# nico-franco-gomez/dsptoolbox

Hardware: AMD Instinct MI355X
Metric: Msamples/s + GB/s vs HBM roofline, 64ch Welch H1 nfft=4096 @1/2/4/8 GPU (higher is better)
Workload: dtype f32

## Files before the change

### dsptoolbox_amd/csrc/kernels_welch4096w.hpp

```cpp
#pragma once
#include <utility>

#include "kernels_welch4096.hpp"

namespace welch4096 {

constexpr int L3S = 17;
constexpr int LDS3_BYTES = 16 * L1S * 8 + 256 * 8 + N * 4;

struct Tw6 {
    float2 a[3];
    float2 b[3];
};

__device__ __forceinline__ void load_tw6(Tw6& tw, const float2* __restrict__ twt, int tid) {
#pragma unroll
    for (int j = 0; j < 3; ++j) {
        tw.a[j] = twt[j * 256 + tid];
        tw.b[j] = twt[(4 * (j + 1) - 1) * 256 + tid];
    }
}

__device__ __forceinline__ void apply_tw6(float2 (&v)[16], const Tw6& tw) {
#pragma unroll
    for (int k1 = 1; k1 < 16; ++k1) {
        const int lo = k1 & 3, hi = k1 >> 2;
        float2 z = v[pos16(k1)];
        if (lo) z = cmul(z, tw.a[lo - 1]);
        if (hi) z = cmul(z, tw.b[hi - 1]);
        v[pos16(k1)] = z;
    }
}

__device__ __forceinline__ __amdgpu_buffer_rsrc_t channel_rsrc(const float* ch, int64_t n_samples) {
    return __builtin_amdgcn_make_buffer_rsrc(const_cast<float*>(ch), 0, (int)(uint32_t)(n_samples * 4), 0x00020000);
}
__device__ __forceinline__ float ld_sample(__amdgpu_buffer_rsrc_t r, int byte_off) {
    return __builtin_bit_cast(float, __builtin_amdgcn_raw_buffer_load_b32(r, byte_off, 0, 0));
}

typedef float v2f_t __attribute__((ext_vector_type(2)));
__device__ __forceinline__ uint32_t lds_addr(const void* p) { return (uint32_t)(uintptr_t)p; }
template <int BYTE_OFF>
__device__ __forceinline__ void lds_rd64(float2& d, uint32_t addr) {
    static_assert(BYTE_OFF >= 0 && BYTE_OFF < 65536 && BYTE_OFF % 8 == 0, "ds_read_b64 offset");
    v2f_t r;
    asm volatile("ds_read_b64 %0, %1 offset:%2" : "=v"(r) : "v"(addr), "n"(BYTE_OFF) : "memory");
    d = make_float2(r.x, r.y);
}
template <int N>
__device__ __forceinline__ void lgkm_wait() {
    static_assert(N >= 0 && N <= 15, "lgkmcnt is a 4-bit counter");
    asm volatile("s_waitcnt lgkmcnt(%0)" ::"n"(N) : "memory");
    __builtin_amdgcn_sched_barrier(0);
}
template <typename F, int... I>
__device__ __forceinline__ void static_for_impl(F&& f, std::integer_sequence<int, I...>) {
    (f(std::integral_constant<int, I>{}), ...);
}
template <int N, typename F>
__device__ __forceinline__ void static_for(F&& f) {
    static_for_impl(static_cast<F&&>(f), std::make_integer_sequence<int, N>{});
}

__device__ __forceinline__ int bin_thread(int tid) { return ((tid & 15) << 4) | (tid >> 4); }

template <typename Hook = NoHook, typename Hook2 = NoHook>
__device__ __forceinline__ void fft4096_w(float2 (&v)[16], const Tw6& tw, float2* __restrict__ buf,
                                          const float2* __restrict__ tw2, int tid,
                                          Hook behind_ex1 = Hook(), Hook2 behind_ex2 = Hook2()) {
    dft16(v);
    apply_tw6(v, tw);
    const int k1u = tid >> 4, n3 = tid & 15;
    __syncthreads();
#pragma unroll
    for (int k1 = 0; k1 < 16; ++k1) buf[k1 * L1S + tid] = v[pos16(k1)];
    float2 w2[15];
#pragma unroll
    for (int k2 = 1; k2 < 16; ++k2) w2[k2 - 1] = tw2[k2 * 16 + n3];
    behind_ex1();
    __syncthreads();
    float2* __restrict__ row = buf + k1u * L1S;
#pragma unroll
    for (int n2 = 0; n2 < 16; ++n2) v[n2] = row[16 * n2 + n3];
    dft16(v);
#pragma unroll
    for (int k2 = 1; k2 < 16; ++k2) v[pos16(k2)] = cmul(v[pos16(k2)], w2[k2 - 1]);
#pragma unroll
    for (int k2 = 0; k2 < 16; ++k2) row[n3 * L3S + k2] = v[pos16(k2)];
    behind_ex2();
    wave_sync();
#pragma unroll
    for (int j = 0; j < 16; ++j) v[j] = row[j * L3S + n3];
    dft16(v);
}

__device__ __forceinline__ void set_prio(int level16, int dither) {
    const int pr = min(3, (level16 + dither) >> 2);
    if (pr == 0)
        __builtin_amdgcn_s_setprio(0);
    else if (pr == 1)
        __builtin_amdgcn_s_setprio(1);
    else if (pr == 2)
        __builtin_amdgcn_s_setprio(2);
    else
        __builtin_amdgcn_s_setprio(3);
}

template <typename LA, typename LB, typename MID = NoHook>
__device__ __forceinline__ void fft4096_wi(float2 (&v)[16], const Tw6& tw, float2* __restrict__ buf,
                                           const float2* __restrict__ tw2, int tid, LA ld_a, LB ld_b,
                                           MID mid = MID()) {
    const int k1u = tid >> 4, n3 = tid & 15;
    float2* __restrict__ col = buf + tid;
    dft16_h(
        v, NoHookI(),
        [&](int g) {
            W4_PIN();
            ld_a(g);
            W4_PIN();
        },
        [&](int g) {
#pragma unroll
        for (int j = 0; j < 4; ++j) {
            float2 z = v[4 * g + j];
            if (g) z = cmul(z, tw.a[g - 1]);
            if (j) z = cmul(z, tw.b[j - 1]);
            W4_PIN();
            col[(g + 4 * j) * L1S] = z;
            W4_PIN();
        }
    });
    __syncthreads();
    mid();
    float2* __restrict__ row = buf + k1u * L1S;
    const uint32_t a_row = lds_addr(row + n3), a_tw2 = lds_addr(tw2 + n3);
    W4_PIN();
    static_for<16>([&](auto ic) {
        constexpr int i = decltype(ic)::value, n2 = 4 * (i & 3) + (i >> 2);
        lds_rd64<16 * n2 * 8>(v[n2], a_row);
    });
    float2 w2[16];
    dft16_h(
        v,
        [&](auto gc) {
            constexpr int g = decltype(gc)::value;
            lgkm_wait<(g == 0 ? 12 : 11)>();
        },
        [&](int g) {
            W4_PIN();
            static_for<4>([&](auto jc) {
                constexpr int j = decltype(jc)::value;
                if (g == 0 && j > 0) lds_rd64<(0 + j) * 16 * 8>(w2[0 + j], a_tw2);
                if (g == 1) lds_rd64<(4 + j) * 16 * 8>(w2[4 + j], a_tw2);
                if (g == 2) lds_rd64<(8 + j) * 16 * 8>(w2[8 + j], a_tw2);
                if (g == 3) lds_rd64<(12 + j) * 16 * 8>(w2[12 + j], a_tw2);
            });
            if (g == 3) lgkm_wait<0>();
            W4_PIN();
        },
        [&](int g) {
#pragma unroll
            for (int j = 0; j < 4; ++j) {
                const int k2 = g + 4 * j;
                float2 z = v[4 * g + j];
                if (k2) z = cmul(z, w2[k2]);
                W4_PIN();
                row[n3 * L3S + k2] = z;
                W4_PIN();
            }
            W4_PIN();
            ld_b(g);
            W4_PIN();
        });
    wave_sync();
    W4_PIN();
    static_for<16>([&](auto ic) {
        constexpr int i = decltype(ic)::value, j = 4 * (i & 3) + (i >> 2);
        lds_rd64<j * L3S * 8>(v[j], a_row);
    });
    dft16_h(
        v,
        [&](auto gc) {
            constexpr int g = decltype(gc)::value;
            lgkm_wait<12 - 4 * g>();
            if (g == 3) __syncthreads();
        },
        NoHookI(), NoHookI());
}

struct Tw6R {
    float2 a[3];
    float2 b[3];
    float2 c;
};
constexpr int TW2R = TWT_R + 4 * 256;

__device__ __forceinline__ void load_tw6r(Tw6R& tw, const float2* __restrict__ twt, int tid) {
#pragma unroll
    for (int j = 0; j < 3; ++j) {
        tw.a[j] = twt[TWT_R + j * 256 + tid];
        tw.b[j] = twt[(4 * (j + 1) - 1) * 256 + tid];
    }
    tw.c = twt[TWT_R + 3 * 256 + tid];
}

__device__ __forceinline__ constexpr int posr16(int k3) { return pos16((16 - k3) & 15); }

template <int R>
__device__ __forceinline__ float2 row_ror(float2 z) {
    if constexpr (R == 0) {
        return z;
    } else {
        const int x = __builtin_amdgcn_update_dpp(0, __float_as_int(z.x), 0x120 + R, 0xf, 0xf, true);
        const int y = __builtin_amdgcn_update_dpp(0, __float_as_int(z.y), 0x120 + R, 0xf, 0xf, true);
        return make_float2(__int_as_float(x), __int_as_float(y));
    }
}

template <typename LA, typename LB>
__device__ __forceinline__ void fft4096_wr(float2 (&v)[16], const Tw6R& tw, float2* __restrict__ buf,
                                           const float2* __restrict__ tw2r, int tid, LA ld_a, LB ld_b) {
    const int k1u = tid >> 4, n3 = tid & 15;
    float2* __restrict__ col = buf + tid;
    dft16_h(
        v, NoHookI(),
        [&](int g) {
            W4_PIN();
            ld_a(g);
            W4_PIN();
        },
        [&](int g) {
#pragma unroll
            for (int j = 0; j < 4; ++j) {
                float2 z = cmul(v[4 * g + j], g ? tw.a[g - 1] : tw.c);
                if (j) z = cmul(z, tw.b[j - 1]);
                W4_PIN();
                col[(g + 4 * j) * L1S] = z;
                W4_PIN();
            }
        });
    __syncthreads();
    const uint32_t a_row = lds_addr(buf + k1u * L1S + n3), a_tw2 = lds_addr(tw2r + n3);
    W4_PIN();
    static_for<16>([&](auto ic) {
        constexpr int i = decltype(ic)::value, n2 = 4 * (i & 3) + (i >> 2);
        lds_rd64<16 * n2 * 8>(v[n2], a_row);
    });
    float2 w2[16];
    dft16_h(
        v,
        [&](auto) {
            lgkm_wait<12>();
        },
        [&](int g) {
            W4_PIN();
            static_for<4>([&](auto jc) {
                constexpr int j = decltype(jc)::value;
                if (g == 0) lds_rd64<(0 + j) * 16 * 8>(w2[0 + j], a_tw2);
                if (g == 1) lds_rd64<(4 + j) * 16 * 8>(w2[4 + j], a_tw2);
                if (g == 2) lds_rd64<(8 + j) * 16 * 8>(w2[8 + j], a_tw2);
                if (g == 3) lds_rd64<(12 + j) * 16 * 8>(w2[12 + j], a_tw2);
            });
            if (g == 3) {
                lgkm_wait<0>();
                __syncthreads();
            }
            W4_PIN();
        },
        [&](int g) {
#pragma unroll
            for (int j = 0; j < 4; ++j) v[4 * g + j] = cmul(v[4 * g + j], w2[g + 4 * j]);
            W4_PIN();
            ld_b(g);
            W4_PIN();
        });
    float2 u[16];
    static_for<16>([&](auto mc) {
        constexpr int m = decltype(mc)::value;
        u[m] = row_ror<m>(v[pos16(m)]);
    });
#pragma unroll
    for (int m = 0; m < 16; ++m) v[m] = u[m];
    dft16(v);
}

__global__ __launch_bounds__(NT) void k_x3(Args p) {
    extern __shared__ __align__(16) float2 lds[];
    float2* buf = lds;
    float2* tw2 = lds + 16 * L1S;
    const int tid = threadIdx.x;
    const int cx = (int)blockIdx.x / p.n_pairs, pr = (int)blockIdx.x - cx * p.n_pairs;
    Tw6R tw;
    float2 v[16];
    {
        Raw<true> raw;
        const __amdgpu_buffer_rsrc_t rs = channel_rsrc(p.sig + (int64_t)cx * p.ld, p.n_samples);
        const int off0 = 4 * (2 * pr * 2048 + tid);
#pragma unroll
        for (int m = 0; m < 24; ++m) raw.s[m] = ld_sample(rs, off0 + 1024 * m);
        float win[16];
        load_tw6r(tw, p.twt, tid);
#pragma unroll
        for (int n1 = 0; n1 < 16; ++n1) win[n1] = p.window[tid + 256 * n1];
        tw2[tid] = p.twt[TW2R + tid];
        window_pair<true>(v, raw, win);
        if (needs_drop(p, pr)) drop_second(v);
    }
    fft4096_wr(v, tw, buf, tw2, tid, NoHookI(), NoHookI());
    if (p.detrend && tid == 0) v[posr16(0)] = make_float2(0.f, 0.f);
    float4* xo = reinterpret_cast<float4*>(p.xs + ((int64_t)cx * p.n_pairs + pr) * N) + tid;
#pragma unroll
    for (int g = 0; g < 8; ++g) {
        float2 z0 = v[posr16(2 * g)], z1 = v[posr16(2 * g + 1)];
        xo[256 * g] = make_float4(z0.x, z0.y, z1.x, z1.y);
    }
    float* pw = reinterpret_cast<float*>(buf);
    const int bt = bin_thread(tid);
    __syncthreads();
#pragma unroll
    for (int k3 = 0; k3 < 16; ++k3) {
        float2 z = v[posr16(k3)];
        pw[fold_pos(bt + 256 * k3)] = z.x * z.x + z.y * z.y;
    }
    __syncthreads();
    float* po = p.px + ((int64_t)cx * p.n_pairs + pr) * NB;
    for (int k = tid; k < NB; k += NT) po[k] = 0.5f * (pw[fold_pos(k)] + pw[fold_pos((N - k) & (N - 1))]);
}

__device__ __forceinline__ void chunk_range(const Args& p, int q, int& p0, int& p1) {
    if (p.use_plus) {
        auto below = [&](int qq) {
            int n = 0;
            for (int w = 0; w < (qq >> 5); ++w) n += __popc(p.plus[w]);
            if (qq & 31) n += __popc(p.plus[qq >> 5] & ((1u << (qq & 31)) - 1u));
            return n;
        };
        const int base = p.n_pairs / p.n_chunks;
        p0 = q * base + below(q);
        p1 = p0 + base + (int)((p.plus[q >> 5] >> (q & 31)) & 1u);
    } else {
        p0 = (int)((int64_t)q * p.n_pairs / p.n_chunks);
        p1 = (int)((int64_t)(q + 1) * p.n_pairs / p.n_chunks);
    }
}

__global__ __launch_bounds__(256) void k_px_sum(Args p) {
    const int q = blockIdx.x, cx = blockIdx.y;
    int p0, p1;
    chunk_range(p, q, p0, p1);
    welchc::px_sum<NB>(p, q, cx, p0, p1);
}

template <bool AUTO = false>
__global__ __launch_bounds__(NT, 3) void k_y3(Args p) {
    extern __shared__ __align__(16) float2 lds[];
    float2* buf = lds;
    float2* tw2 = lds + 16 * L1S;
    float* winl = reinterpret_cast<float*>(lds + 16 * L1S + 256);
    const int tid = threadIdx.x;
    int q, c;
    {
        const int b = blockIdx.x, total = p.n_chunks * p.n_ch;
        const int u = (total & 7) == 0 ? (b & 7) * (total >> 3) + (b >> 3) : b;
        q = u / p.n_ch;
        c = u - q * p.n_ch;
    }
    Tw6R tw;
    load_tw6r(tw, p.twt, tid);
    tw2[tid] = p.twt[TW2R + tid];
#pragma unroll
    for (int n1 = 0; n1 < 16; ++n1) winl[tid + 256 * n1] = p.window[tid + 256 * n1];
    const float* ch = p.sig + (int64_t)c * p.ld;
    int p0, p1;
    chunk_range(p, q, p0, p1);
    const int cx = p.n_cx > 1 ? c : 0;
    if (!AUTO && p.n_cx <= 1) {
        double* red = reinterpret_cast<double*>(lds);
        const int bpc = (NB + p.n_ch - 1) / p.n_ch;
        const int b0 = c * bpc, b1 = min(b0 + bpc, NB);
        const int lw = bpc <= 32 ? 5 : (bpc <= 64 ? 6 : (bpc <= 128 ? 7 : 8)), width = 1 << lw, rows = NT >> lw;
        const int rg = tid >> lw, kl = tid & (width - 1);
        for (int kb = b0; kb < b1; kb += width) {
            const int k = kb + kl;
            double sum = 0.0;
            if (k < b1)
                for (int pr = p0 + rg; pr < p1; pr += rows) sum += (double)p.px[(int64_t)pr * NB + k];
            red[rg * width + kl] = sum;
            __syncthreads();
            if (rg == 0 && k < b1) {
                double t = 0.0;
                for (int j = 0; j < rows; ++j) t += red[j * width + kl];
                p.psx[(int64_t)q * NB + k] = (float)t;
            }
            __syncthreads();
        }
    }
    float2 T[16];
    float P[16];
#pragma unroll
    for (int j = 0; j < 16; ++j) {
        T[j] = make_float2(0.f, 0.f);
        P[j] = 0.f;
    }
    float carry[8], nx[16];
    const __amdgpu_buffer_rsrc_t rs = channel_rsrc(ch, p.n_samples);
    const __amdgpu_buffer_rsrc_t xrs =
        AUTO ? rs
             : __builtin_amdgcn_make_buffer_rsrc(const_cast<float2*>(p.xs + ((int64_t)cx * p.n_pairs + p0) * N), 0,
                                                 (int)(uint32_t)((p1 - p0) * (N * 8)), 0x00020000);
    if (p0 < p1) {
        const int off0 = 4 * (2 * p0 * 2048 + tid);
#pragma unroll
        for (int j = 0; j < 8; ++j) carry[j] = ld_sample(rs, off0 + 1024 * j);
#pragma unroll
        for (int j = 0; j < 16; ++j) nx[j] = ld_sample(rs, off0 + 1024 * (8 + j));
    }
    float winr[16];
#pragma unroll
    for (int n1 = 0; n1 < 16; ++n1) winr[n1] = winl[tid + 256 * n1];
    for (int pr = p0; pr < p1; ++pr) {
        float2 v[16];
        const int level16 = ((p1 - pr - 1) * 16) / (p1 - p0);
        set_prio(level16, (pr * 5) & 3);
#pragma unroll
        for (int n1 = 0; n1 < 16; ++n1) {
            const float w = winr[n1];
            const float a = n1 < 8 ? carry[n1] : nx[n1 - 8];
            v[n1] = make_float2(a * w, nx[n1] * w);
        }
#pragma unroll
        for (int j = 0; j < 8; ++j) carry[j] = nx[8 + j];
        if (needs_drop(p, pr)) drop_second(v);
        float2 xw[16];
        const int off1 = 4 * ((2 * pr + 2) * 2048 + tid) + 1024 * 8;
        const int xoff = (pr - p0) * (N * 8) + tid * 16;
        fft4096_wr(
            v, tw, buf, tw2, tid,
            [&](int g) {
#pragma unroll
                for (int j = 0; j < 4; ++j) nx[4 * g + j] = ld_sample(rs, off1 + 1024 * (4 * g + j));
            },
            [&](int g) {
                if (!AUTO) {
#pragma unroll
                    for (int j = 0; j < 2; ++j) {
                        const float4 q4 =
                            __builtin_bit_cast(float4, __builtin_amdgcn_raw_buffer_load_b128(xrs, xoff + 4096 * (2 * g + j), 0, 0));
                        xw[2 * (2 * g + j)] = make_float2(q4.x, q4.y);
                        xw[2 * (2 * g + j) + 1] = make_float2(q4.z, q4.w);
                    }
                }
            });
#pragma unroll
        for (int k3 = 0; k3 < 16; ++k3) {
            float2 z = v[posr16(k3)];
            if (!AUTO) {
                float2 w = xw[k3];
                T[k3].x = fmaf(w.x, z.x, fmaf(w.y, z.y, T[k3].x));
                T[k3].y = fmaf(w.x, z.y, fmaf(-w.y, z.x, T[k3].y));
            }
            P[k3] = fmaf(z.x, z.x, fmaf(z.y, z.y, P[k3]));
        }
        __builtin_amdgcn_sched_barrier(0);
#pragma unroll
        for (int n1 = 0; n1 < 16; ++n1) winr[n1] = winl[tid + 256 * n1];
        __builtin_amdgcn_sched_barrier(0);
    }
    if (p.detrend && tid == 0) P[0] = 0.f;
    const int bt = bin_thread(tid);
    __syncthreads();
    const int64_t so = ((int64_t)q * p.n_ch + c) * NB;
    if (!AUTO) {
#pragma unroll
        for (int k3 = 0; k3 < 16; ++k3) buf[fold_pos(bt + 256 * k3)] = T[k3];
        __syncthreads();
        for (int k = tid; k < NB; k += NT) {
            float2 a = buf[fold_pos(k)], b = buf[fold_pos((N - k) & (N - 1))];
            p.pxy[so + k] = make_float2(0.5f * (a.x + b.x), 0.5f * (a.y - b.y));
        }
        __syncthreads();
    }
    float* pw = reinterpret_cast<float*>(buf);
#pragma unroll
    for (int k3 = 0; k3 < 16; ++k3) pw[fold_pos(bt + 256 * k3)] = P[k3];
    __syncthreads();
    for (int k = tid; k < NB; k += NT) p.pyy[so + k] = 0.5f * (pw[fold_pos(k)] + pw[fold_pos((N - k) & (N - 1))]);
}

inline int chunks_for3(int n_pairs, int n_ch, int want = 0) {
    if (want <= 0) {
        want = (768 + n_ch - 1) / n_ch;
        const int by_len = (n_pairs + 63) / 64;
        if (want < by_len) want = by_len;
        for (int w = want; w < want + 8; ++w)
            if (((int64_t)w * n_ch) % 8 == 0) {
                want = w;
                break;
            }
    }
    if (want > n_pairs) want = n_pairs;
    if (want < 1) want = 1;
    return want;
}
inline Plan plan3(int n_frames, int n_cy, int want_chunks = 0) {
    Plan pl;
    pl.n_pairs = (n_frames + 1) / 2;
    pl.n_chunks = chunks_for3(pl.n_pairs, n_cy, want_chunks);
    pl.ppc = (pl.n_pairs + pl.n_chunks - 1) / pl.n_chunks;
    return pl;
}
inline void place_remainder(Args& a, int n_ch) {
    a.use_plus = 0;
    for (auto& w : a.plus) w = 0;
    const int nc = a.n_chunks, total = nc * n_ch;
    if (nc > 24 * 32 || (total & 7) != 0 || nc <= 0) return;
    const int base = a.n_pairs / nc, rem = a.n_pairs - base * nc;
    a.use_plus = 1;
    if (rem == 0) return;
    const int U = total / 8;
    std::vector<int> ov((size_t)8 * nc, 0);
    for (int u = 0; u < total; ++u) ov[(size_t)(u / U) * nc + u / n_ch] += 1;
    std::vector<int64_t> load(8, 0);
    for (int x = 0; x < 8; ++x)
        for (int q = 0; q < nc; ++q) load[x] += (int64_t)ov[(size_t)x * nc + q] * base;
    std::vector<char> taken(nc, 0);
    for (int r = 0; r < rem; ++r) {
        int best = -1;
        int64_t best_max = 0, best_aff = 0;
        for (int q = 0; q < nc; ++q) {
            if (taken[q]) continue;
            int64_t mx = 0, aff = 0;
            for (int x = 0; x < 8; ++x) {
                const int64_t l = load[x] + ov[(size_t)x * nc + q];
                mx = std::max(mx, l);
                if (ov[(size_t)x * nc + q]) aff = std::max(aff, l);
            }
            if (best < 0 || mx < best_max || (mx == best_max && aff < best_aff)) {
                best = q;
                best_max = mx;
                best_aff = aff;
            }
        }
        taken[best] = 1;
        a.plus[best >> 5] |= 1u << (best & 31);
        for (int x = 0; x < 8; ++x) load[x] += ov[(size_t)x * nc + best];
    }
}

inline bool fits3(int64_t n_samples, int n_frames) {
    return n_samples < ((int64_t)1 << 30) - 8192 && (int64_t)(n_frames + 2) * 2048 < ((int64_t)1 << 30) - 8192;
}

}
```

Baseline: 650,900.

## Fuse cross-spectrum accumulation into final DFT stage and keep window in registers

Adds a finish hook to the last radix-16 stage of the 4096-point FFT, so the cross-spectrum and power accumulation for each group runs as soon as that group is ready. The X-spectrum loads are split into two 4-element buffers that are refilled as they are used, which cuts register pressure from holding 16 values. The window now stays in registers instead of being staged in LDS and reloaded every iteration, which removes the LDS window region. The stage-2 twiddle reads are also reordered and spread across groups with finer lgkm waits. The k_x3 output store changes to index v directly, which relies on the new output ordering of the FFT.

```diff
diff --git a/dsptoolbox_amd/csrc/kernels_welch4096w.hpp b/dsptoolbox_amd/csrc/kernels_welch4096w.hpp
--- a/dsptoolbox_amd/csrc/kernels_welch4096w.hpp
+++ b/dsptoolbox_amd/csrc/kernels_welch4096w.hpp
@@ -6,7 +6,7 @@
 namespace welch4096 {
 
 constexpr int L3S = 17;
-constexpr int LDS3_BYTES = 16 * L1S * 8 + 256 * 8 + N * 4;
+constexpr int LDS3_BYTES = 16 * L1S * 8 + 256 * 8;
 
 struct Tw6 {
     float2 a[3];
@@ -218,9 +218,9 @@
     }
 }
 
-template <typename LA, typename LB>
+template <typename LA, typename LB, typename LC = NoHookI>
 __device__ __forceinline__ void fft4096_wr(float2 (&v)[16], const Tw6R& tw, float2* __restrict__ buf,
-                                           const float2* __restrict__ tw2r, int tid, LA ld_a, LB ld_b) {
+                                           const float2* __restrict__ tw2r, int tid, LA ld_a, LB ld_b, LC fin = LC()) {
     const int k1u = tid >> 4, n3 = tid & 15;
     float2* __restrict__ col = buf + tid;
     dft16_h(
@@ -250,17 +250,16 @@
     float2 w2[16];
     dft16_h(
         v,
-        [&](auto) {
-            lgkm_wait<12>();
+        [&](auto gc) {
+            constexpr int g = decltype(gc)::value;
+            lgkm_wait<(g == 3 ? 8 : 12)>();
         },
         [&](int g) {
             W4_PIN();
             static_for<4>([&](auto jc) {
                 constexpr int j = decltype(jc)::value;
-                if (g == 0) lds_rd64<(0 + j) * 16 * 8>(w2[0 + j], a_tw2);
-                if (g == 1) lds_rd64<(4 + j) * 16 * 8>(w2[4 + j], a_tw2);
-                if (g == 2) lds_rd64<(8 + j) * 16 * 8>(w2[8 + j], a_tw2);
-                if (g == 3) lds_rd64<(12 + j) * 16 * 8>(w2[12 + j], a_tw2);
+                if (g == 0) lds_rd64<(0 + 4 * j) * 16 * 8>(w2[0 + 4 * j], a_tw2);
+                if (g == 1) lds_rd64<(1 + 4 * j) * 16 * 8>(w2[1 + 4 * j], a_tw2);
             });
             if (g == 3) {
                 lgkm_wait<0>();
@@ -269,9 +268,16 @@
             W4_PIN();
         },
         [&](int g) {
+            if (g == 2) lgkm_wait<4>();
+            if (g == 3) lgkm_wait<0>();
 #pragma unroll
             for (int j = 0; j < 4; ++j) v[4 * g + j] = cmul(v[4 * g + j], w2[g + 4 * j]);
             W4_PIN();
+            static_for<4>([&](auto jc) {
+                constexpr int j = decltype(jc)::value;
+                if (g == 0) lds_rd64<(2 + 4 * j) * 16 * 8>(w2[2 + 4 * j], a_tw2);
+                if (g == 1) lds_rd64<(3 + 4 * j) * 16 * 8>(w2[3 + 4 * j], a_tw2);
+            });
             ld_b(g);
             W4_PIN();
         });
@@ -282,7 +288,14 @@
     });
 #pragma unroll
     for (int m = 0; m < 16; ++m) v[m] = u[m];
-    dft16(v);
+    dft16_h(v, NoHookI(), NoHookI(), [&](int g) {
+        W4_PIN();
+        if (g == 0) fin(std::integral_constant<int, 0>{});
+        if (g == 1) fin(std::integral_constant<int, 1>{});
+        if (g == 2) fin(std::integral_constant<int, 2>{});
+        if (g == 3) fin(std::integral_constant<int, 3>{});
+        W4_PIN();
+    });
 }
 
 __global__ __launch_bounds__(NT) void k_x3(Args p) {
@@ -307,13 +320,13 @@
         window_pair<true>(v, raw, win);
         if (needs_drop(p, pr)) drop_second(v);
     }
-    fft4096_wr(v, tw, buf, tw2, tid, NoHookI(), NoHookI());
+    fft4096_wr(v, tw, buf, tw2, tid, NoHookI(), NoHookI(), NoHookI());
     if (p.detrend && tid == 0) v[posr16(0)] = make_float2(0.f, 0.f);
     float4* xo = reinterpret_cast<float4*>(p.xs + ((int64_t)cx * p.n_pairs + pr) * N) + tid;
 #pragma unroll
-    for (int g = 0; g < 8; ++g) {
-        float2 z0 = v[posr16(2 * g)], z1 = v[posr16(2 * g + 1)];
-        xo[256 * g] = make_float4(z0.x, z0.y, z1.x, z1.y);
+    for (int i = 0; i < 8; ++i) {
+        float2 z0 = v[2 * i], z1 = v[2 * i + 1];
+        xo[256 * i] = make_float4(z0.x, z0.y, z1.x, z1.y);
     }
     float* pw = reinterpret_cast<float*>(buf);
     const int bt = bin_thread(tid);
@@ -357,7 +370,6 @@
     extern __shared__ __align__(16) float2 lds[];
     float2* buf = lds;
     float2* tw2 = lds + 16 * L1S;
-    float* winl = reinterpret_cast<float*>(lds + 16 * L1S + 256);
     const int tid = threadIdx.x;
     int q, c;
     {
@@ -369,8 +381,9 @@
     Tw6R tw;
     load_tw6r(tw, p.twt, tid);
     tw2[tid] = p.twt[TW2R + tid];
-#pragma unroll
-    for (int n1 = 0; n1 < 16; ++n1) winl[tid + 256 * n1] = p.window[tid + 256 * n1];
+    float win[16];
+#pragma unroll
+    for (int n1 = 0; n1 < 16; ++n1) win[n1] = p.window[tid + 256 * n1];
     const float* ch = p.sig + (int64_t)c * p.ld;
     int p0, p1;
     chunk_range(p, q, p0, p1);
@@ -416,25 +429,31 @@
 #pragma unroll
         for (int j = 0; j < 16; ++j) nx[j] = ld_sample(rs, off0 + 1024 * (8 + j));
     }
-    float winr[16];
-#pragma unroll
-    for (int n1 = 0; n1 < 16; ++n1) winr[n1] = winl[tid + 256 * n1];
     for (int pr = p0; pr < p1; ++pr) {
         float2 v[16];
         const int level16 = ((p1 - pr - 1) * 16) / (p1 - p0);
         set_prio(level16, (pr * 5) & 3);
 #pragma unroll
         for (int n1 = 0; n1 < 16; ++n1) {
-            const float w = winr[n1];
+            const float w = win[n1];
             const float a = n1 < 8 ? carry[n1] : nx[n1 - 8];
             v[n1] = make_float2(a * w, nx[n1] * w);
         }
 #pragma unroll
         for (int j = 0; j < 8; ++j) carry[j] = nx[8 + j];
         if (needs_drop(p, pr)) drop_second(v);
-        float2 xw[16];
+        float2 xe[4], xo[4];
         const int off1 = 4 * ((2 * pr + 2) * 2048 + tid) + 1024 * 8;
         const int xoff = (pr - p0) * (N * 8) + tid * 16;
+        auto ld_x = [&](float2(&x)[4], int g) {
+#pragma unroll
+            for (int h = 0; h < 2; ++h) {
+                const float4 q4 =
+                    __builtin_bit_cast(float4, __builtin_amdgcn_raw_buffer_load_b128(xrs, xoff + 4096 * (2 * g + h), 0, 0));
+                x[2 * h] = make_float2(q4.x, q4.y);
+                x[2 * h + 1] = make_float2(q4.z, q4.w);
+            }
+        };
         fft4096_wr(
             v, tw, buf, tw2, tid,
             [&](int g) {
@@ -443,29 +462,29 @@
             },
             [&](int g) {
                 if (!AUTO) {
-#pragma unroll
-                    for (int j = 0; j < 2; ++j) {
-                        const float4 q4 =
-                            __builtin_bit_cast(float4, __builtin_amdgcn_raw_buffer_load_b128(xrs, xoff + 4096 * (2 * g + j), 0, 0));
-                        xw[2 * (2 * g + j)] = make_float2(q4.x, q4.y);
-                        xw[2 * (2 * g + j) + 1] = make_float2(q4.z, q4.w);
+                    if (g == 2) ld_x(xe, 0);
+                    if (g == 3) ld_x(xo, 1);
+                }
+            },
+            [&](auto gc) {
+                constexpr int g = decltype(gc)::value;
+                float2(&x)[4] = (g & 1) ? xo : xe;
+#pragma unroll
+                for (int j = 0; j < 4; ++j) {
+                    const int k3 = (16 - (g + 4 * j)) & 15;
+                    float2 z = v[4 * g + j];
+                    if (!AUTO) {
+                        float2 w = x[j];
+                        T[k3].x = fmaf(w.x, z.x, fmaf(w.y, z.y, T[k3].x));
+                        T[k3].y = fmaf(w.x, z.y, fmaf(-w.y, z.x, T[k3].y));
                     }
+                    P[k3] = fmaf(z.x, z.x, fmaf(z.y, z.y, P[k3]));
+                }
+                if (!AUTO && g < 2) {
+                    W4_PIN();
+                    ld_x(x, g + 2);
                 }
             });
-#pragma unroll
-        for (int k3 = 0; k3 < 16; ++k3) {
-            float2 z = v[posr16(k3)];
-            if (!AUTO) {
-                float2 w = xw[k3];
-                T[k3].x = fmaf(w.x, z.x, fmaf(w.y, z.y, T[k3].x));
-                T[k3].y = fmaf(w.x, z.y, fmaf(-w.y, z.x, T[k3].y));
-            }
-            P[k3] = fmaf(z.x, z.x, fmaf(z.y, z.y, P[k3]));
-        }
-        __builtin_amdgcn_sched_barrier(0);
-#pragma unroll
-        for (int n1 = 0; n1 < 16; ++n1) winr[n1] = winl[tid + 256 * n1];
-        __builtin_amdgcn_sched_barrier(0);
     }
     if (p.detrend && tid == 0) P[0] = 0.f;
     const int bt = bin_thread(tid);
```

Result: no change. 653,100, median of 6 (+0.3%).
